# Rose-STL-Lab/spherical-dyffusion

Measured on AMD Instinct MI355X. Metric: forecast-steps/sec (180x360, 63ch), 25-member ensemble DYffusion sampling, whole job, higher is better.
Workload: dtype f32 tensors; every GEMM-class kernel (1x1 convs, fused MLP, Legendre analysis/synthesis, dhconv) as 3-pass split-f16 MFMA with f32 accumulation; FFT / norms / pointwise in f32 (statistics f64); 1 GPU; 25-member ensemble x horizon-6 DYffusion sampling pass (6 forecaster + 10 interpolator SFNO forwards, dropout stream on, AR feedback), 180x360, 63 state + 2 forcing channels, embed 256, 8 blocks; horizon=6, relayed_members=0, parallelism=members of one initial condition sharded over GPUs, no data-path collective

## Files before the change

spherical-dyffusion_amd/csrc/capi.hip:

```cpp
#include <cmath>
#include <cstdio>
#include <cstdlib>
#include <cstring>
#include <mutex>
#include <string>
#include <vector>

#include "common.h"
#include "fft.h"
#include "pointwise.h"

static inline int round_up(int v, int m) { return (v + m - 1) / m * m; }
static inline size_t round_up_sz(size_t v, size_t m) { return (v + m - 1) / m * m; }

template <class F>
static float h3_pack_host(std::vector<_Float16>& buf, int nb, int rows, int K, int rows_pad, int Kpad, F value) {
  float mx = 0.f;
  for (int b = 0; b < nb; ++b)
    for (int r = 0; r < rows; ++r)
      for (int k = 0; k < K; ++k) mx = std::fmax(mx, std::fabs(value(b, r, k)));
  const float s = sdy_h3_scale(mx);
  const size_t plane = (size_t)nb * rows_pad * Kpad;
  buf.assign(2 * plane, (_Float16)0.0f);
  for (int b = 0; b < nb; ++b)
// ... 50 lines not shown
  float* d_pct = nullptr;
  float* d_tw = nullptr;
  float* d_pw = nullptr;
  SdyFftDesc fft;
  int gemm_mode = 0;
  void* d_wq_h3 = nullptr;
  void* d_pct_h3 = nullptr;
  float s_wq = 1.f, s_pct = 1.f;
  int h3_rows_fwd = 0, h3_k_fwd = 0, h3_rows_inv = 0, h3_k_inv = 0;
  void* d_wq_frag = nullptr;
  void* d_pct_frag = nullptr;
  float s_wq_frag = 1.f, s_pct_frag = 1.f;
  void* d_wq_par = nullptr;
  void* d_pct_par = nullptr;
  float s_wq_par = 1.f, s_pct_par = 1.f;
  int* d_kdead = nullptr;
  int* d_mcut = nullptr;
  enum Leg { LEG_PAR, LEG_H3, LEG_GEMM_H3, LEG_GEMM_F32 } leg = LEG_GEMM_F32;
  bool fused360 = false;
};

namespace {
struct SdySwitches {
  bool gemm_f32, no_fft360, no_leg_par, no_leg_frag, no_dh_frag, no_fused_mlp, no_drop_skip, no_skip_fold;
};
const SdySwitches& sw() {
  static const SdySwitches v = [] {
    auto on = [](const char* n) { return std::getenv(n) != nullptr; };
    const char* g = std::getenv("SDY_GEMM_MODE");
    return SdySwitches{g && std::string(g) == "f32", on("SDY_NO_FFT360"), on("SDY_NO_LEG_PAR"), on("SDY_NO_LEG_FRAG"),
                       on("SDY_NO_DH_FRAG"), on("SDY_NO_FUSED_MLP"), on("SDY_NO_DROP_SKIP"), on("SDY_NO_SKIP_FOLD")};
  }();
  return v;
}
}
static int env_gemm_mode() { return sw().gemm_f32 ? 0 : 1; }

template <class D, class T>
static hipError_t upload(D** dst, const std::vector<T>& v) {
  hipError_t e = hipMalloc((void**)dst, v.size() * sizeof(T));
  return e == hipSuccess ? hipMemcpy(*dst, v.data(), v.size() * sizeof(T), hipMemcpyHostToDevice) : e;
}
struct LegTables { const float *wqT, *pf; int nlat, lmax, Lpad4, Kpad4; };
static float leg_wq_at(void* c, int m, int l, int k) {
  const LegTables* x = static_cast<const LegTables*>(c);
  return x->wqT[((size_t)m * x->nlat + k) * x->Lpad4 + l];
}
static float leg_pct_at(void* c, int m, int k, int l) {
  const LegTables* x = static_cast<const LegTables*>(c);
  return x->pf[((size_t)m * x->lmax + l) * x->Kpad4 + k];
}

extern "C" int sdy_sht_plan_create(int nlat, int nlon, int lmax, int mmax, int grid, sdy_sht_plan** out) {
  return sdy_sht_plan_create_ex(nlat, nlon, lmax, mmax, grid, env_gemm_mode(), out);
// ... 420 lines not shown
  if (!(p->fft.fft360 && p->fft.n == 180) || C % 16 != 0) return SDY_ERR_UNSUPPORTED;
  if (!tiled_stride_ok(zt_bstride, C, p->nlat * p->nlon)) return SDY_ERR_ARG;
  return sdy_fft360_launch_inv(p->fft, Yf, bias, nullptr, B, C, p->nlat, p->mtr, 0, nullptr, (hipStream_t)stream, zt, zt_bstride,
                               part);
}

static inline int h3_mpad(int Cout) { return Cout > 128 ? round_up(Cout, 256) : 128; }
static inline int h3_kpad(int Cin) { return round_up(Cin, 64); }

extern "C" size_t sdy_h3_pack_bytes(int Cout, int Cin) {
  if (Cout <= 0 || Cin <= 0) return 0;
  return (size_t)2 * h3_mpad(Cout) * h3_kpad(Cin) * sizeof(_Float16);
}

extern "C" int sdy_h3_pack_weight(const float* w, int Cout, int Cin, void* packed_dev, float* scale) {
  if (!w || !packed_dev || !scale || Cout <= 0 || Cin <= 0) return SDY_ERR_ARG;
  std::vector<_Float16> buf;
  *scale = h3_pack_host(buf, 1, Cout, Cin, h3_mpad(Cout), h3_kpad(Cin),
                        [&](int, int o, int i) { return w[(size_t)o * Cin + i]; });
  SDY_HIP_TRY(hipMemcpy(packed_dev, buf.data(), buf.size() * sizeof(_Float16), hipMemcpyHostToDevice));
  return SDY_OK;
}

extern "C" int sdy_conv1x1(const sdy_conv_args* a, void* stream) {
  if (!a || !a->x || (!a->wt && !a->w_h3 && !a->w_frag) || !a->out) return SDY_ERR_ARG;
  if (a->B <= 0 || a->Cin <= 0 || a->Cout <= 0 || a->HW <= 0) return SDY_ERR_ARG;
  if (!a->w_h3 && a->ldw < a->Cout) return SDY_ERR_ARG;
  if ((a->pa == nullptr) != (a->pd == nullptr)) return SDY_ERR_ARG;
  if (a->add_mode != 0 && !a->add) return SDY_ERR_ARG;
  if ((!a->w_h3 && (a->ldw & 3)) || (a->HW & 3) || (a->x_bstride & 3) || (a->out_bstride & 3)) return SDY_ERR_ALIGN;
  if (a->drop_p < 0.0f || a->drop_p >= 1.0f) return SDY_ERR_ARG;
  if (a->w_frag && sdy_conv256_h3_supported(a->Cin, a->Cout) && a->drop_p == 0.0f && !a->keep_mask && !a->batch_scale)
    return sdy_conv256_h3_launch(a, (hipStream_t)stream);
  if (a->stats || a->out_tiled || a->x_rows) return SDY_ERR_UNSUPPORTED;
  GemmParams g{};
  g.A = a->wt; g.lda = a->ldw; g.sA = 0;
  g.B = a->x; g.ldb = a->HW; g.sB = a->x_bstride;
  g.C = a->out; g.ldc = a->HW; g.sC = a->out_bstride;
  g.M = round_up(a->Cout, 4); g.M_store = a->Cout; g.N = a->HW; g.K = a->Cin; g.nbatch = a->B;
  g.tile = a->Cout > 64 ? SDY_TILE_128x128 : SDY_TILE_64x128;
  g.tag = (a->kernel_tag >= 1 && a->kernel_tag <= 3) ? a->kernel_tag : 0;
  g.pa = a->pa; g.pd = a->pd; g.p_bstride = a->Cin;
  g.bias = a->bias;
  g.add = a->add_mode ? a->add : nullptr; g.sAdd = a->add_bstride; g.ldadd = a->HW; g.add_mode = a->add_mode;
  g.act = a->act;
  if (a->drop_p > 0.0f) {
    g.drop_thr = sdy_drop_threshold16(a->drop_p);
    if (g.drop_thr == 0u) g.drop_thr = 1u;
    g.drop_scale = 1.0f / (1.0f - a->drop_p);
    g.keep_mask = a->keep_mask;
  }
  g.seed_lo = (uint32_t)(a->seed & 0xFFFFFFFFu); g.seed_hi = (uint32_t)(a->seed >> 32);
  g.stream_id = a->stream_id; g.call = a->call; g.batch_offset = a->batch_offset;
  if (a->rows_per_call < 0 || (a->rows_per_call > 0 && a->B % a->rows_per_call)) return SDY_ERR_ARG;
  g.rows_per_call = a->rows_per_call > 0 ? a->rows_per_call : a->B;
  g.batch_scale = a->batch_scale;
  if (a->w_h3) {
    const int Mp = h3_mpad(a->Cout), Kp = h3_kpad(a->Cin);
    return sdy_gemm_h3_launch(g, a->w_h3, Mp, Kp, 0, (long)Mp * Kp, a->w_h3_scale, 0, (hipStream_t)stream);
  }
  return sdy_gemm_launch(g, (hipStream_t)stream);
}

extern "C" int sdy_cold_update(const float* x_s, const float* x_ip_next, const float* x_ip_s, float* out, size_t n,
                               void* stream) {
  return sdy_cold_update_launch(x_s, x_ip_next, x_ip_s, out, n, (hipStream_t)stream);
}

extern "C" int sdy_concat_channels(const float* const* src, const int* chans, int nsrc, float* out, int B, int HW,
                                   void* stream) {
  if (!src || !chans || nsrc < 1 || nsrc > 4) return SDY_ERR_ARG;
  long total = 0;
  for (int i = 0; i < nsrc; ++i) total += chans[i];
  return sdy_concat_launch(src, chans, nsrc, out, total * HW, B, HW, (hipStream_t)stream);
}

extern "C" int sdy_cond_noise_fill(uint64_t seed, uint32_t call, uint32_t batch_offset, int rows_per_call, int B, int C, int HW,
                                   float* out, void* stream) {
  return sdy_cond_noise_launch(seed, call, batch_offset, rows_per_call, B, C, HW, out, (hipStream_t)stream);
}

namespace {

struct DevBuf {
  float* p = nullptr;
// ... 33 lines not shown
  if (c.gemm_mode != 1) return DH_GEMM_F32;
  if (!sdy_dhconv_frag_supported(c.embed_dim, c.embed_dim) || sw().no_dh_frag) return DH_GEMM_H3;
  return skip_foldable(c, i) && !sw().no_skip_fold ? DH_FOLDED : DH_FRAG;
}

namespace {
struct XfSide {
  const sdy_sht_plan* plan;
  bool polar;
  bool tiled;
  int ilv;
  const int* mcut;
};

struct BlockPath {
  XfSide in, out;
  bool scale_residual;
  bool fused_mlp;
  bool lazy_norm;
  bool cs_tiled;
  DhKind dh;
  enum Skip { SKIP_CONV, SKIP_GELU, SKIP_IN_FFT } skip;
  bool stats1;
  bool z_tiled;
  bool drop_skip;
};
}

struct sdy_sfno {
  sdy_sfno_config cfg;
  int HW, catC, decC, ldo;
  sdy_sht_plan* plan_data = nullptr;
  sdy_sht_plan* plan_lg = nullptr;
  DevBuf pos, e0w, e0b, e2w, d0w, d0b, d2w;
  struct Pair { std::vector<float> w1_host, w2_host; void* w = nullptr; float s1 = 1.0f, s2 = 1.0f; } enc, dec;
  DevBuf t1w, t1b, t3w, t3b, freq, wbt, bb;
  std::vector<BlockW> blk;
  std::vector<BlockPath> path;
  SdyTimeMlp tm;
  std::string missing;
  const float* enc_ws = nullptr;
  int enc_B = 0;
  bool enc_has_stats = false;
};

static int dev_alloc(DevBuf& b, size_t n) {
// ... 276 lines not shown
    if (rest == "mlp.fwd.2.bias" || rest == "mlp.fwd.3.bias") { EXPECT_NUMEL(E); return dev_upload(w.b2, host, numel); }
  }
  return SDY_ERR_NAME;
}

static BlockPath resolve_path(const sdy_sfno* n, int i) {
  const sdy_sfno_config& c = n->cfg;
  const BlockW& w = n->blk[i];
  const int E = c.embed_dim, ilv = spec_ilv(c);
  auto side = [&](const sdy_sht_plan* p) {
    const bool polar = plan_polar_ok(p, E), tiled = plan_tiled_ok(p, E, ilv);
    return XfSide{p, polar, tiled, tiled ? 2 : ilv, polar ? p->d_mcut : nullptr};
  };
  BlockPath b;
  b.in = side(i == 0 ? n->plan_data : n->plan_lg);
  b.out = side(i == c.num_layers - 1 ? n->plan_data : n->plan_lg);
  b.scale_residual = b.in.plan != b.out.plan;
  b.fused_mlp = w.mlp && !sw().no_fused_mlp;
  b.lazy_norm = b.fused_mlp && !b.scale_residual;
  b.dh = dhconv_kind(c, i);
  const bool dh_frag = b.dh == DH_FOLDED || b.dh == DH_FRAG;
  b.cs_tiled = b.in.tiled && b.out.tiled && dh_frag && b.in.plan->lmax == b.out.plan->lmax && b.in.plan->mtr == b.out.plan->mtr;
  b.stats1 = c.gemm_mode == 1 && w.skw.frag && sdy_conv256_h3_supported(E, E);
  b.z_tiled = b.stats1 && b.fused_mlp;
  b.skip = b.dh != DH_FOLDED ? BlockPath::SKIP_CONV : (b.out.tiled && b.z_tiled) ? BlockPath::SKIP_IN_FFT : BlockPath::SKIP_GELU;
  b.drop_skip = b.fused_mlp && b.z_tiled && b.cs_tiled && !sw().no_drop_skip;
  return b;
}

extern "C" int sdy_sfno_ready(const sdy_sfno* n_c) {
  sdy_sfno* n = const_cast<sdy_sfno*>(n_c);
  if (!n) return SDY_ERR_ARG;
  if (!n->path.empty()) return SDY_OK;
  const sdy_sfno_config& c = n->cfg;
  n->missing.clear();
  auto need = [&](const DevBuf& b, const std::string& nm) {
    if (!b.set && n->missing.empty()) n->missing = nm;
  };
  if (c.pos_embed) need(n->pos, "pos_embed");
  need(n->e0w, "encoder.0.weight"); need(n->e0b, "encoder.0.bias"); need(n->e2w, "encoder.2.weight");
  need(n->d0w, "decoder.0.weight"); need(n->d0b, "decoder.0.bias"); need(n->d2w, "decoder.2.weight");
  if (c.with_time_emb) {
    need(n->t1w, "time_emb_mlp.1.weight"); need(n->t1b, "time_emb_mlp.1.bias");
    need(n->t3w, "time_emb_mlp.3.weight"); need(n->t3b, "time_emb_mlp.3.bias");
  }
  for (int i = 0; i < c.num_layers; ++i) {
// ... 393 lines not shown
      SDY_STAGE_N(ST_FFT_INV, k.Bp, sdy_fft_launch_inv(pout->fft, Xf, bias, y, k.Bp, E, pout->nlat, pout->mtr, P.out.ilv,
                                                       P.out.mcut, stream));
    return SDY_OK;
  }

  int inner_skip(const Blk& k) {
    const BlockPath& P = k.P;
    const BlockW& bw = k.w;
    if (P.skip == BlockPath::SKIP_IN_FFT) {
      SDY_STAGE_N(ST_NORM_COEFFS, k.Bp, sdy_instnorm_from_partials_launch(sp, P.out.plan->nlat, k.Bp, E, HW, bw.n1w.p, bw.n1b.p,
                                                                          1e-6f, ca1, cd1, stream));
      return SDY_OK;
    }
    if (P.skip == BlockPath::SKIP_GELU) {
      SDY_STAGE_N(ST_SKIP_GELU, k.Bp, sdy_gelu_stats_launch(y, xbs, k.z, k.z_bs, P.z_tiled ? 1 : 0, st1, k.Bp, E, HW, stream));
    } else {
      sdy_conv_args cv = conv_args(bw.skw, k.Bp);
      cv.x_rows = P.lazy_norm ? k.rows : nullptr;
      cv.x = P.lazy_norm ? cur : xn; cv.x_bstride = xbs;
      if (P.lazy_norm) { cv.pa = ca; cv.pd = cd; }
      cv.ldw = E; cv.out = k.z; cv.out_bstride = k.z_bs; cv.out_tiled = P.z_tiled ? 1 : 0;
      cv.Cin = E; cv.Cout = E; cv.bias = bw.skb.p; cv.add = y; cv.add_bstride = xbs; cv.add_mode = 1; cv.act = 1; cv.kernel_tag = 3;
      if (P.stats1) cv.stats = st1;
      SDY_STAGE_N(ST_SKIP_CONV, k.Bp, sdy_conv1x1(&cv, stream));
    }
    if (P.skip == BlockPath::SKIP_GELU || P.stats1)
      SDY_STAGE_N(ST_NORM_COEFFS, k.Bp, sdy_instnorm_from_stats(st1, k.Bp, E, HW, bw.n1w.p, bw.n1b.p, nullptr, 0, 1e-6f, ca1, cd1,
                                                                stream));
    else
      SDY_STAGE(ST_NORM_COEFFS, sdy_instnorm_coeffs_launch(y, B, E, HW, bw.n1w.p, bw.n1b.p, nullptr, 0, 1e-6f, ca1, cd1, stream));
    return SDY_OK;
  }

  int mlp(const Blk& k) {
    const BlockW& bw = k.w;
    const int i = k.i, Hd = c.mlp_hidden;
    const float* dps = (drop && n->tm.dp_rate[i] > 0.f) ? dp + (size_t)i * B : nullptr;
    const float* keep1 = (pm > 0.f && a->keep_masks) ? a->keep_masks[2 * i] : nullptr;
    const float* keep2 = (pm > 0.f && a->keep_masks) ? a->keep_masks[2 * i + 1] : nullptr;
    if (k.P.fused_mlp) {
      sdy_mlp_args ma;
      std::memset(&ma, 0, sizeof(ma));
      ma.x = k.z; ma.x_bstride = k.z_bs; ma.x_tiled = k.P.z_tiled ? 1 : 0; ma.pa = ca1; ma.pd = cd1;
      ma.w = bw.mlp; ma.w1_scale = bw.mlp_s1; ma.w2_scale = bw.mlp_s2; ma.b1 = bw.b1.p; ma.b2 = bw.b2.p;
      ma.out = k.dst; ma.out_bstride = k.dst_bs;
      if (k.P.lazy_norm) { ma.add = cur; ma.add_bstride = xbs; ma.add_a = ca; ma.add_d = cd; }
      else { ma.add = xn; ma.add_bstride = xbs; ma.add_by_launch_row = k.rows ? 1 : 0; }
// ... 65 lines not shown
```

spherical-dyffusion_amd/csrc/common.h:

```cpp
#pragma once
#include <hip/hip_runtime.h>
#include <stdint.h>
#include <atomic>
#include <cmath>
#include <type_traits>

#include "../../include/sdy_amd.h"

#define SDY_HIP_TRY(expr)                       \
  do {                                          \
    hipError_t _e = (expr);                     \
    if (_e != hipSuccess) return (int)_e;       \
  } while (0)

#define SDY_TRY(expr)             \
  do {                            \
    int _r = (expr);              \
    if (_r != SDY_OK) return _r;  \
  } while (0)

static inline int sdy_launch_status() {
  hipError_t e = hipGetLastError();
  return e == hipSuccess ? SDY_OK : (int)e;
}
// ... 274 lines not shown
  int M_store;
  int lda, ldb, ldc;
  long sA, sB, sC;
  int nbatch;
  int a_kcontig;
  int b_cplx;
  int cplx_Ei, cplx_Eo;
  int tri_mode, tri_B;
  int tile;
  int tag;
  const float* pa; const float* pd; long p_bstride;
  const float* bias;
  const float* add; long sAdd; int ldadd; int add_mode;
  int act;
  uint32_t drop_thr; float drop_scale; const float* keep_mask;
  uint32_t seed_lo, seed_hi, stream_id, call, batch_offset;
  int rows_per_call;
  const float* batch_scale;
};
int sdy_gemm_launch(const GemmParams& p, hipStream_t stream);
int sdy_gemm_h3_launch(const GemmParams& p, const void* packed, int rows_pad, int Kpad, long bstride, long plane_halfs,
                       float w_scale, int rows_mode, hipStream_t stream);

int sdy_conv256_h3_launch(const sdy_conv_args* a, hipStream_t stream);
extern "C" int sdy_conv256_h3_pack_cin(const float* w_host, int Cin, void* dev, float* scale);
extern "C" size_t sdy_conv256_h3_pack_bytes_cin(int Cin);
int sdy_dh_h3_pack(const float* w_host, int L, void* packed_dev, float* scale, int ilv);
int sdy_dh_h3_launch(const float* Cs_in, const void* packed, float scale, float* Cs_out, int L, int mtr, int B, int ilv,
                      hipStream_t stream, int tiled = 0, int B_in = 0);

typedef float (*sdy_leg_value_fn)(void* ctx, int z, int row, int k);
int sdy_leg_h3_supported(int rows, int K);
size_t sdy_leg_h3_table_bytes(int nz);
int sdy_leg_h3_pack(int nz, int rows, int K, sdy_leg_value_fn value, void* ctx, void* dev, float* scale);
int sdy_leg_par_supported(int nlat, int lmax);
size_t sdy_leg_par_table_bytes(int nz);
int sdy_leg_par_pack(int nz, int nlat, int lmax, int fwd, sdy_leg_value_fn value, void* ctx, void* dev, float* scale);
int sdy_leg_par_launch(const void* table, float scale, int nz, const float* X, long ldx, long sX, float* C, long ldc,
                       long sC, int rows_out, int K, int N, int fwd, const int* kdead, hipStream_t stream, long tsx = 0, long tsc = 0);
int sdy_leg_h3_launch(const void* table, float scale, int nz, const float* X, long ldx, long sX, float* C, long ldc, long sC,
                      int M_store, int K, int N, int tri, hipStream_t stream);

int sdy_factor_radices(int n, int* radices, int* nstages);
```

spherical-dyffusion_amd/csrc/conv_h3.hip:

```cpp
#include <cmath>
#include <cstdlib>
#include <type_traits>
#include <vector>

#include "common.h"

namespace {

constexpr int CE = 256;
constexpr int CTN = 64;
constexpr int CKMAX = 384;
constexpr int CRING = 4;
constexpr float CSX = SDY_ACT_SX;
constexpr int CSTAT_BYTES = CE * 2 * 8;
#ifndef SDY_CONV_STAMP_T0
#define SDY_CONV_STAMP_T0 2
#endif

template <int KBLK, int NW>
struct ConvCfg {
  static_assert(NW == 4 || NW == 8, "4 or 8 waves");
  static constexpr int NT = 64 * NW;
  static constexpr int MT = 8 / NW;
  static constexpr int RS = 4 * NW;
// ... 16 lines not shown
  const float* x; long x_bs;
  const float* pa; const float* pd;
  const sdy_f16x8* w;
  const float* bias;
  const float* add; long add_bs; int add_mode;
  int act;
  float* out; long out_bs;
  int out_tiled;
  double* stats;
  int HW, B;
  int Cin;
  float out_scale;
  unsigned* flags;
  unsigned* head;
  const float* gelu_tab;
  SdyImgMap xmap;
  unsigned long long* stamps;
};

__device__ __forceinline__ int cv_swz(int px) { return (px & 15) ^ (((px >> 4) & 1) * 3); }
template <int KROW>
__device__ __forceinline__ int cv_off(int px, int c) { return px * KROW + (((c & ~15) | ((c ^ cv_swz(px)) & 15)) << 3); }

template <int KBLK, int NW>
__global__ __launch_bounds__(64 * NW, NW == 4 ? 2 : 1) void conv_h3_kernel(const ConvParams p) {
  using G = ConvCfg<KBLK, NW>;
  constexpr int CMT = G::MT, CRS = G::RS, COC = G::OC, CRPT = G::RPT, KROW = G::KROW, CGPK = G::GPK, CGPW = G::GPW;
  __shared__ __attribute__((aligned(16))) unsigned char smem[G::LDS_BYTES];
  _Float16* Xs_hi = reinterpret_cast<_Float16*>(smem);
  _Float16* Xs_lo = Xs_hi + CTN * KROW;
  float* Os = reinterpret_cast<float*>(smem);

  const int tid = threadIdx.x, lane = tid & 63, wave = tid >> 6;
  int h = lane >> 5, l31 = lane & 31;
  int q0 = tid & 15, o0 = tid >> 4;
  const int tpi = (p.HW + CTN - 1) / CTN;
  const int ntiles = tpi * p.B;
  const int t_per = (ntiles + (int)gridDim.x - 1) / (int)gridDim.x;
  const int t_begin = (int)blockIdx.x * t_per;
  const int t_end = (t_begin + t_per < ntiles) ? t_begin + t_per : ntiles;

  sdy_f16x8 r_hi[CRING], r_lo[CRING];
  constexpr int CGROUP_BYTES = SDY_GROUP * (int)sizeof(sdy_f16x8);
  const char* const wbase = reinterpret_cast<const char*>(p.w) + (size_t)__builtin_amdgcn_readfirstlane(wave) * CGPW * CGROUP_BYTES;
  unsigned woff = (unsigned)lane * 16u;
#pragma unroll
  for (int s = 0; s < CRING; ++s) {
    r_hi[s] = sdy_ring_ld(wbase, woff, 0);
    r_lo[s] = sdy_ring_ld(wbase, woff, CGROUP_BYTES / 2);
    woff += CGROUP_BYTES;
  }
  constexpr int NWIN = KBLK * CMT;
  if (NWIN == 1) woff -= CRING * CGROUP_BYTES;

  double* Ss = reinterpret_cast<double*>(smem + G::TILE_BYTES);
  float* Bs = reinterpret_cast<float*>(smem + G::TILE_BYTES + CSTAT_BYTES);
  if (tid < CE) {
    Bs[tid] = p.bias ? p.bias[tid] / p.out_scale : 0.0f;
    Ss[2 * tid] = 0.0; Ss[2 * tid + 1] = 0.0;
  }
  float* Gt = reinterpret_cast<float*>(smem + G::TILE_BYTES + CSTAT_BYTES + CE * 4);
  const unsigned gt_base = (unsigned)(uintptr_t)Gt;
  const bool tab_gelu = SDY_CONV_GELU_TAB && p.act == 1;
  if (tab_gelu) gelu_tab_to_lds(Gt, p.gelu_tab, tid, G::NT, 1.0f / SDY_GELU_SX);
  const float os_scale = tab_gelu ? p.out_scale * SDY_GELU_WS : p.out_scale;

  f32x4 xr[COC][8], addv[CRPT];
  auto img = [&](const float* base, long bs, int t) { return base + (long)(t / tpi) * bs; };
  auto ximg = [&](int t) { return p.x + (long)sdy_img(p.xmap, t / tpi) * p.x_bs; };
  auto lane_col = [&](int t) {
    const int nn = (t % tpi) * CTN + 4 * q0;
    return nn < p.HW ? nn : 0;
  };
  const float* addsrc = p.add ? p.add : p.out;
  const long addsrc_bs = p.add ? p.add_bs : p.out_bs;
  if (t_begin < t_end) {
    const float* xz = ximg(t_begin);
    const unsigned xo = (unsigned)(8 * o0 * p.HW + lane_col(t_begin)) * 4u;
#pragma unroll
    for (int oc = 0; oc < COC; ++oc)
#pragma unroll
      for (int e = 0; e < 8; ++e) {
        const int ch = 8 * (o0 + CRS * oc) + e;
        xr[oc][e] = f32x4{0.f, 0.f, 0.f, 0.f};
        if (ch < p.Cin) xr[oc][e] = sdy_ld16s(xz + (long)(8 * CRS * oc + e) * p.HW, xo);
      }
  }

  for (int tile = t_begin; tile < t_end; ++tile) {
    asm volatile("" : "+v"(l31), "+v"(h), "+v"(q0), "+v"(o0));
    const int tile_it = tile - t_begin;
    auto stamp = [&](int i) {
      if (SDY_STAMPS_ON && p.stamps && blockIdx.x == 3 && tid == 0 && tile_it >= SDY_CONV_STAMP_T0 && tile_it < SDY_CONV_STAMP_T0 + 4)
        p.stamps[(tile_it - SDY_CONV_STAMP_T0) * 8 + i] = __builtin_amdgcn_s_memtime();
    };
    stamp(0);
    const int z = tile / tpi;
    const int zx = sdy_img(p.xmap, z);
    const int n0 = (tile - z * tpi) * CTN;
    const bool full = n0 + CTN <= p.HW;

    {
      float amax = 0.0f;
      const bool ok = full || (n0 + 4 * q0 < p.HW);
#pragma unroll
      for (int oc = 0; oc < COC; ++oc) {
        const int c0 = 8 * (o0 + CRS * oc);
        if (8 * CRS * oc + 8 * CRS > KROW && c0 >= KROW) continue;
        float av[8], dv[8];
        if (p.pa) {
          const f32x4 a0 = *reinterpret_cast<const f32x4*>(p.pa + (long)zx * CE + c0);
          const f32x4 a1 = *reinterpret_cast<const f32x4*>(p.pa + (long)zx * CE + c0 + 4);
          const f32x4 d0 = *reinterpret_cast<const f32x4*>(p.pd + (long)zx * CE + c0);
          const f32x4 d1 = *reinterpret_cast<const f32x4*>(p.pd + (long)zx * CE + c0 + 4);
#pragma unroll
          for (int e = 0; e < 4; ++e) {
            av[e] = a0[e] * CSX; av[e + 4] = a1[e] * CSX;
            dv[e] = d0[e] * CSX; dv[e + 4] = d1[e] * CSX;
          }
        } else {
#pragma unroll
          for (int e = 0; e < 8; ++e) { av[e] = CSX; dv[e] = 0.f; }
        }
#pragma unroll
        for (int pp = 0; pp < 4; ++pp) {
          sdy_f16x8 vh, vl;
          float v[8];
#pragma unroll
          for (int e = 0; e < 8; ++e) v[e] = (ok && c0 + e < p.Cin) ? fmaf(xr[oc][e][pp], av[e], dv[e]) : 0.0f;
          sdy_split8(v, vh, vl, amax);
          const int off = cv_off<KROW>(4 * q0 + pp, o0 + CRS * oc);
          *reinterpret_cast<sdy_f16x8*>(Xs_hi + off) = vh;
          *reinterpret_cast<sdy_f16x8*>(Xs_lo + off) = vl;
        }
      }
      sdy_flag_range(p.flags, amax, p.head);
    }
    __syncthreads();
    stamp(1);
    const int col = n0 + 4 * q0;
    const bool c_ok = full || col < p.HW;
    const unsigned ro = (unsigned)(o0 * p.HW + (c_ok ? col : 0)) * 4u;
    const unsigned ro_out = p.out_tiled ? (unsigned)(o0 * CTN + 4 * q0) * 4u : ro;
    const int out_rs = p.out_tiled ? CTN : p.HW;
    const int tnext = (tile + 1 < t_end) ? tile + 1 : tile;
    const float* xz_next = ximg(tnext);
    const unsigned xo_next = (unsigned)(8 * o0 * p.HW + lane_col(tnext)) * 4u;
    stamp(2);
    f32x16 acc[CMT][2];
#pragma unroll
    for (int mi = 0; mi < CMT; ++mi)
#pragma unroll
      for (int r4 = 0; r4 < 4; ++r4) {
        const f32x4 b4 = *reinterpret_cast<const f32x4*>(Bs + 32 * (CMT * wave + mi) + 8 * r4 + 4 * h);
#pragma unroll
        for (int j = 0; j < 2; ++j)
#pragma unroll
          for (int r = 0; r < 4; ++r) acc[mi][j][4 * r4 + r] = b4[r];
      }
#pragma unroll
    for (int kb = 0; kb < KBLK; ++kb) {
#pragma unroll
      for (int i = 0; i < 4; ++i) {
        const int ks = 4 * kb + i;
        sdy_f16x8 bh[2], bl[2];
#pragma unroll
        for (int j = 0; j < 2; ++j) {
          const int off = cv_off<KROW>(32 * j + l31, 2 * ks + h);
          bh[j] = *reinterpret_cast<const sdy_f16x8*>(Xs_hi + off);
          bl[j] = *reinterpret_cast<const sdy_f16x8*>(Xs_lo + off);
        }
#pragma unroll
        for (int mi = 0; mi < CMT; ++mi) {
          const int g = kb * CGPK + CMT * i + mi;
          const int s = g % CRING;
#pragma unroll
          for (int j = 0; j < 2; ++j) SDY_CROSS_TERM(acc[mi][j] = __builtin_amdgcn_mfma_f32_32x32x16_f16(r_lo[s], bh[j], acc[mi][j], 0, 0, 0));
#pragma unroll
          for (int j = 0; j < 2; ++j) SDY_CROSS_TERM(acc[mi][j] = __builtin_amdgcn_mfma_f32_32x32x16_f16(r_hi[s], bl[j], acc[mi][j], 0, 0, 0));
#pragma unroll
          for (int j = 0; j < 2; ++j) acc[mi][j] = __builtin_amdgcn_mfma_f32_32x32x16_f16(r_hi[s], bh[j], acc[mi][j], 0, 0, 0);
          r_hi[s] = sdy_ring_ld(wbase, woff, 0);
          r_lo[s] = sdy_ring_ld(wbase, woff, CGROUP_BYTES / 2);
          woff += CGROUP_BYTES;
          if ((g + CRING + 1) % (NWIN * CRING) == 0) woff -= NWIN * CRING * CGROUP_BYTES;
          __builtin_amdgcn_sched_barrier(0);
        }
      }
    }

    stamp(3);
    {
      const float* az = img(addsrc, addsrc_bs, tile);
#pragma unroll
      for (int i = 0; i < CRPT; ++i) addv[i] = p.add ? sdy_ld16s(az + (long)(CRS * i) * p.HW, ro) : f32x4{0.f, 0.f, 0.f, 0.f};
    }
    __syncthreads();
    stamp(4);
#pragma unroll
    for (int mi = 0; mi < CMT; ++mi)
#pragma unroll
      for (int j = 0; j < 2; ++j)
#pragma unroll
        for (int r = 0; r < 16; ++r) {
          const int row = 32 * (CMT * wave + mi) + (r & 3) + 8 * (r >> 2) + 4 * h;
          Os[row * CTN + 32 * j + l31] = acc[mi][j][r] * os_scale;
        }
    __syncthreads();
    stamp(5);
    {
      float* oz = p.out + (long)z * p.out_bs + (p.out_tiled ? (long)(tile - z * tpi) * (CE * CTN) : 0L);
#pragma unroll
      for (int i = 0; i < CRPT; ++i) {
        f32x4 v = *reinterpret_cast<const f32x4*>(Os + (o0 + CRS * i) * CTN + 4 * q0);
        if (tab_gelu) {
          if (p.add_mode == 1) v = addv[i] * SDY_GELU_WS + v;
          v = f32x4{gelu_tab16(v.x, gt_base), gelu_tab16(v.y, gt_base), gelu_tab16(v.z, gt_base), gelu_tab16(v.w, gt_base)};
        } else {
        if (p.add_mode == 1) v += addv[i];
        if (p.act == 1) {
          const sdy_gf2 g0 = gelu_erf2(sdy_gf2{v.x, v.y}), g1 = gelu_erf2(sdy_gf2{v.z, v.w});
          v = f32x4{g0.x, g0.y, g1.x, g1.y};
        }
        }
        if (p.add_mode == 2) v += addv[i];
        if (c_ok) sdy_st16s(oz + (long)(CRS * i) * out_rs, ro_out, v);
#pragma unroll
        for (int k = 0; k < G::PPI; ++k) {
          const int piece = G::PPI * i + k, oc = piece >> 3, e = piece & 7;
          if (oc < COC) {
            const int ch = 8 * (o0 + CRS * oc) + e;
            if (ch < p.Cin) xr[oc][e] = sdy_ld16s(xz_next + (long)(8 * CRS * oc + e) * p.HW, xo_next);
          }
        }
        if (p.stats) {
          const float s1 = row16_sum(c_ok ? (v.x + v.y) + (v.z + v.w) : 0.0f);
          const float s2 = row16_sum(c_ok ? (v.x * v.x + v.y * v.y) + (v.z * v.z + v.w * v.w) : 0.0f);
          if (q0 == 0) {
            double* st = Ss + 2 * (o0 + CRS * i);
            __hip_atomic_fetch_add(st, (double)s1, __ATOMIC_RELAXED, __HIP_MEMORY_SCOPE_WORKGROUP);
            __hip_atomic_fetch_add(st + 1, (double)s2, __ATOMIC_RELAXED, __HIP_MEMORY_SCOPE_WORKGROUP);
          }
        }
      }
    }
    stamp(6);
    {
      const int nt = tile + 1;
      if (p.stats && (nt >= t_end || nt / tpi != z)) {
        __syncthreads();
        if (tid < CE) {
          double* st = p.stats + ((long)z * CE + tid) * 2;
          __hip_atomic_fetch_add(st, Ss[2 * tid], __ATOMIC_RELAXED, __HIP_MEMORY_SCOPE_AGENT);
          __hip_atomic_fetch_add(st + 1, Ss[2 * tid + 1], __ATOMIC_RELAXED, __HIP_MEMORY_SCOPE_AGENT);
          Ss[2 * tid] = 0.0; Ss[2 * tid + 1] = 0.0;
        }
      }
    }
    stamp(7);
    __syncthreads();
// ... 31 lines not shown
extern "C" int sdy_conv256_h3_pack_cin(const float* w_host, int Cin, void* dev, float* scale) {
  if (!w_host || !dev || !scale || Cin < 1 || Cin > CKMAX) return SDY_ERR_ARG;
  const float s = sdy_h3_scale(sdy_h3_absmax(w_host, (size_t)CE * Cin));
  int nw, ksw, mt;
  conv_layout(Cin, &nw, &ksw, &mt);
  const size_t gh = (size_t)SDY_GROUP * 8;
  std::vector<_Float16> buf((size_t)nw * mt * ksw * gh);
  _Float16* d = buf.data();
  for (int w = 0; w < nw; ++w)
    for (int ks = 0; ks < ksw; ++ks)
      for (int mi = 0; mi < mt; ++mi, d += gh)
        sdy_h3_put_group(d, s, [&](int r, int k) {
          const int kk = 16 * ks + k;
          return kk < Cin ? w_host[(size_t)(32 * (mt * w + mi) + r) * Cin + kk] : 0.0f;
        });
  SDY_HIP_TRY(hipMemcpy(dev, buf.data(), buf.size() * sizeof(_Float16), hipMemcpyHostToDevice));
  *scale = s;
  return SDY_OK;
}
extern "C" int sdy_conv256_h3_pack(const float* w_host, void* dev, float* scale) {
  return sdy_conv256_h3_pack_cin(w_host, CE, dev, scale);
}

template <int KBLK, int NW>
static void conv_launch(const ConvParams& p, long ntiles, int n_cu, hipStream_t stream) {
  using G = ConvCfg<KBLK, NW>;
  const long want = (long)n_cu * G::WGS;
  dim3 grid((unsigned)(ntiles < want ? ntiles : want));
  hipLaunchKernelGGL((conv_h3_kernel<KBLK, NW>), grid, dim3(G::NT), 0, stream, p);
}

int sdy_conv256_h3_launch(const sdy_conv_args* a, hipStream_t stream) {
  if (!a || !a->x || !a->w_frag || !a->out || a->B <= 0 || a->HW <= 0) return SDY_ERR_ARG;
  if (!sdy_conv256_h3_supported(a->Cin, a->Cout)) return SDY_ERR_UNSUPPORTED;
  if (a->drop_p > 0.f || a->keep_mask || a->batch_scale) return SDY_ERR_UNSUPPORTED;
  if (a->pa && a->Cin != CE) return SDY_ERR_UNSUPPORTED;
  if ((a->HW & 3) || (a->x_bstride & 3) || (a->out_bstride & 3) || (a->add_mode && (a->add_bstride & 3))) return SDY_ERR_ALIGN;
  if ((long)a->HW * CKMAX * 4 >= (1L << 32)) return SDY_ERR_UNSUPPORTED;
  ConvParams p;
  p.x = a->x; p.x_bs = a->x_bstride; p.pa = a->pa; p.pd = a->pd;
  p.w = reinterpret_cast<const sdy_f16x8*>(a->w_frag);
  p.bias = a->bias;
  p.add = a->add_mode ? a->add : nullptr; p.add_bs = a->add_bstride; p.add_mode = a->add_mode;
  p.act = a->act;
  p.out = a->out; p.out_bs = a->out_bstride; p.out_tiled = a->out_tiled;
  if (a->out_tiled && a->add_mode && a->add == a->out) return SDY_ERR_ARG;
  p.stats = a->stats;
  SDY_TRY(sdy_flags_ptr(&p.flags));
  SDY_TRY(sdy_headroom_ptr(SDY_RANGE_CONV, &p.head));
  SDY_TRY(sdy_gelu_table_ptr(&p.gelu_tab));
  p.HW = a->HW; p.B = a->B; p.Cin = a->Cin;
  SDY_TRY(sdy_img_map_fill(p.xmap, a->x_rows, a->B));
  p.out_scale = 1.0f / (a->w_frag_scale * CSX);
  p.stamps = nullptr;
#if SDY_STAMPS_ON
  if (std::getenv("SDY_CONV_STAMPS")) {
    if (!g_cstamps) SDY_HIP_TRY(hipMalloc(&g_cstamps, 64 * sizeof(unsigned long long)));
    p.stamps = g_cstamps;
  }
#endif
  int n_cu = 0;
  SDY_TRY(sdy_cu_count(&n_cu));
  const long ntiles = (long)((a->HW + CTN - 1) / CTN) * a->B;
  switch ((a->Cin + 63) / 64) {
    case 1: conv_launch<1, 4>(p, ntiles, n_cu, stream); break;
    case 2: conv_launch<2, 4>(p, ntiles, n_cu, stream); break;
    case 3: conv_launch<3, 4>(p, ntiles, n_cu, stream); break;
    case 4: conv_launch<4, 4>(p, ntiles, n_cu, stream); break;
    case 5: conv_launch<5, 8>(p, ntiles, n_cu, stream); break;
    default: conv_launch<6, 8>(p, ntiles, n_cu, stream); break;
  }
  return sdy_launch_status();
}
```

spherical-dyffusion_amd/ops.py:

```python
from __future__ import annotations

import ctypes as C
from typing import Optional

import torch

from ._lib import SdyConvArgs, SdyMlpArgs, SdyPairArgs, aligned, check, current_stream, lib, ptr


def _f32c(t: torch.Tensor) -> torch.Tensor:
    if not t.is_cuda:
        raise RuntimeError("sdy_amd ops run on the GPU only (no CPU fallback)")
    return aligned(t.to(torch.float32).contiguous())


def _aux(t: torch.Tensor, dev) -> torch.Tensor:
    return t.detach().to(dev, torch.float32).contiguous()


def contract_dhconv(x: torch.Tensor, weight: torch.Tensor, separable: bool = False,
                    operator_type: str = "dhconv", gemm_mode: Optional[str] = None) -> torch.Tensor:
    if separable or operator_type != "dhconv":
        raise NotImplementedError("only the non-separable dhconv contraction is on the hot path")
    B, Ci, L, M = x.shape
# ... 29 lines not shown
    out = out * tri[None, None, :, :, None]
    return torch.view_as_complex(out.contiguous())


def instnorm_coeffs(x: torch.Tensor, gamma: torch.Tensor, beta: torch.Tensor,
                    scale_shift: Optional[torch.Tensor] = None, eps: float = 1e-6):
    x = _f32c(x)
    B, Cc, H, W = x.shape
    a = torch.empty(B, Cc, dtype=torch.float32, device=x.device)
    d = torch.empty_like(a)
    g, b_ = _aux(gamma, x.device), _aux(beta, x.device)
    ss = _aux(scale_shift, x.device) if scale_shift is not None else None
    with torch.cuda.device(x.device):
        check(lib.sdy_instnorm_coeffs(ptr(x), B, Cc, H * W, ptr(g), ptr(b_), ptr(ss), 2 * Cc, eps, ptr(a), ptr(d),
                                      current_stream()), "sdy_instnorm_coeffs")
    return a, d


def conv1x1(x: torch.Tensor, weight: torch.Tensor, bias: Optional[torch.Tensor] = None, *,
            pre_affine=None, add: Optional[torch.Tensor] = None, add_mode: int = 0, gelu: bool = False,
            drop_p: float = 0.0, keep_mask: Optional[torch.Tensor] = None, seed: int = 0, call: int = 0,
            stream_id: int = 0, batch_offset: int = 0, batch_scale: Optional[torch.Tensor] = None,
            kernel_tag: int = 0, out: Optional[torch.Tensor] = None, wt_prepared=None, h3: bool = False,
            h3_prepared=None, frag_prepared=None, stats: Optional[torch.Tensor] = None) -> torch.Tensor:
    x = _f32c(x)
    B, Cin, H, W = x.shape
    w2 = weight.detach().to(torch.float32).reshape(weight.shape[0], -1)
    Cout = w2.shape[0]
    assert w2.shape[1] == Cin
    ldw = (Cout + 3) // 4 * 4
    if wt_prepared is not None:
        wt = wt_prepared
    else:
        wt = torch.zeros(Cin, ldw, dtype=torch.float32, device=x.device)
        wt[:, :Cout] = w2.t().to(x.device)
    if out is None:
        out = torch.empty(B, Cout, H, W, dtype=torch.float32, device=x.device)
    a = SdyConvArgs()
    a.x, a.x_bstride = ptr(x), Cin * H * W
    a.wt, a.ldw = ptr(wt), ldw
    a.out, a.out_bstride = ptr(out), Cout * H * W
    a.B, a.Cin, a.Cout, a.HW = B, Cin, Cout, H * W
    keep = [x, wt, out]
    if h3 or h3_prepared is not None:
        if h3_prepared is None:
            h3_prepared = pack_h3(w2, x.device)
        a.w_h3, a.w_h3_scale = ptr(h3_prepared[0]), h3_prepared[1]
        keep.append(h3_prepared[0])
    if pre_affine is not None:
        pa, pd = _aux(pre_affine[0], x.device), _aux(pre_affine[1], x.device)
        a.pa, a.pd = ptr(pa), ptr(pd)
        keep += [pa, pd]
    if bias is not None:
        bb = _aux(bias, x.device)
        a.bias = ptr(bb)
        keep.append(bb)
    if add is not None:
        ad = _aux(add, x.device)
        a.add = ptr(ad)
        a.add_bstride = 0 if ad.shape[0] == 1 and B > 1 else Cout * H * W
        a.add_mode = add_mode
        keep.append(ad)
    a.act = 1 if gelu else 0
    a.drop_p = drop_p
# ... 328 lines not shown
```

Baseline: 159.9 member-forecast-steps/s.

## Add weight-stationary 8-wave variant of the 256-channel split-f16 skip conv

Adds a weight-stationary specialization of the 256x256 conv_h3 kernel that runs on 8 waves. Each wave keeps its full slice of hi/lo weight fragments in registers for the whole K sweep, and B fragments from LDS are double-buffered across k-steps. The add and gelu/residual form is hard-wired, the residual load is moved before the MFMA loop, and the next tile's input is prefetched after it. This targets the skip conv in each block to cut repeated weight-ring reloads, at the cost of higher register pressure and one workgroup per CU. The Python wrapper also gains x_rows and out_tiled arguments.

```diff
diff --git a/spherical-dyffusion_amd/csrc/capi.hip b/spherical-dyffusion_amd/csrc/capi.hip
--- a/spherical-dyffusion_amd/csrc/capi.hip
+++ b/spherical-dyffusion_amd/csrc/capi.hip
@@ -96,14 +96,15 @@
 
 namespace {
 struct SdySwitches {
-  bool gemm_f32, no_fft360, no_leg_par, no_leg_frag, no_dh_frag, no_fused_mlp, no_drop_skip, no_skip_fold;
+  bool gemm_f32, no_fft360, no_leg_par, no_leg_frag, no_dh_frag, no_fused_mlp, no_drop_skip, no_skip_fold, no_conv_ws;
 };
 const SdySwitches& sw() {
   static const SdySwitches v = [] {
     auto on = [](const char* n) { return std::getenv(n) != nullptr; };
     const char* g = std::getenv("SDY_GEMM_MODE");
     return SdySwitches{g && std::string(g) == "f32", on("SDY_NO_FFT360"), on("SDY_NO_LEG_PAR"), on("SDY_NO_LEG_FRAG"),
-                       on("SDY_NO_DH_FRAG"), on("SDY_NO_FUSED_MLP"), on("SDY_NO_DROP_SKIP"), on("SDY_NO_SKIP_FOLD")};
+                       on("SDY_NO_DH_FRAG"), on("SDY_NO_FUSED_MLP"), on("SDY_NO_DROP_SKIP"), on("SDY_NO_SKIP_FOLD"),
+                       on("SDY_NO_CONV_WS")};
   }();
   return v;
 }
@@ -570,7 +571,7 @@
   return SDY_OK;
 }
 
-extern "C" int sdy_conv1x1(const sdy_conv_args* a, void* stream) {
+static int conv1x1(const sdy_conv_args* a, void* stream, bool conv_ws) {
   if (!a || !a->x || (!a->wt && !a->w_h3 && !a->w_frag) || !a->out) return SDY_ERR_ARG;
   if (a->B <= 0 || a->Cin <= 0 || a->Cout <= 0 || a->HW <= 0) return SDY_ERR_ARG;
   if (!a->w_h3 && a->ldw < a->Cout) return SDY_ERR_ARG;
@@ -579,7 +580,7 @@
   if ((!a->w_h3 && (a->ldw & 3)) || (a->HW & 3) || (a->x_bstride & 3) || (a->out_bstride & 3)) return SDY_ERR_ALIGN;
   if (a->drop_p < 0.0f || a->drop_p >= 1.0f) return SDY_ERR_ARG;
   if (a->w_frag && sdy_conv256_h3_supported(a->Cin, a->Cout) && a->drop_p == 0.0f && !a->keep_mask && !a->batch_scale)
-    return sdy_conv256_h3_launch(a, (hipStream_t)stream);
+    return sdy_conv256_h3_launch(a, (hipStream_t)stream, conv_ws ? 1 : 0);
   if (a->stats || a->out_tiled || a->x_rows) return SDY_ERR_UNSUPPORTED;
   GemmParams g{};
   g.A = a->wt; g.lda = a->ldw; g.sA = 0;
@@ -609,6 +610,7 @@
   }
   return sdy_gemm_launch(g, (hipStream_t)stream);
 }
+extern "C" int sdy_conv1x1(const sdy_conv_args* a, void* stream) { return conv1x1(a, stream, !sw().no_conv_ws); }
 
 extern "C" int sdy_cold_update(const float* x_s, const float* x_ip_next, const float* x_ip_s, float* out, size_t n,
                                void* stream) {
@@ -688,6 +690,7 @@
   DhKind dh;
   enum Skip { SKIP_CONV, SKIP_GELU, SKIP_IN_FFT } skip;
   bool stats1;
+  bool conv_ws;
   bool z_tiled;
   bool drop_skip;
 };
@@ -1010,6 +1013,7 @@
   const bool dh_frag = b.dh == DH_FOLDED || b.dh == DH_FRAG;
   b.cs_tiled = b.in.tiled && b.out.tiled && dh_frag && b.in.plan->lmax == b.out.plan->lmax && b.in.plan->mtr == b.out.plan->mtr;
   b.stats1 = c.gemm_mode == 1 && w.skw.frag && sdy_conv256_h3_supported(E, E);
+  b.conv_ws = b.stats1 && !sw().no_conv_ws;
   b.z_tiled = b.stats1 && b.fused_mlp;
   b.skip = b.dh != DH_FOLDED ? BlockPath::SKIP_CONV : (b.out.tiled && b.z_tiled) ? BlockPath::SKIP_IN_FFT : BlockPath::SKIP_GELU;
   b.drop_skip = b.fused_mlp && b.z_tiled && b.cs_tiled && !sw().no_drop_skip;
@@ -1449,7 +1453,7 @@
       cv.ldw = E; cv.out = k.z; cv.out_bstride = k.z_bs; cv.out_tiled = P.z_tiled ? 1 : 0;
       cv.Cin = E; cv.Cout = E; cv.bias = bw.skb.p; cv.add = y; cv.add_bstride = xbs; cv.add_mode = 1; cv.act = 1; cv.kernel_tag = 3;
       if (P.stats1) cv.stats = st1;
-      SDY_STAGE_N(ST_SKIP_CONV, k.Bp, sdy_conv1x1(&cv, stream));
+      SDY_STAGE_N(ST_SKIP_CONV, k.Bp, conv1x1(&cv, stream, P.conv_ws));
     }
     if (P.skip == BlockPath::SKIP_GELU || P.stats1)
       SDY_STAGE_N(ST_NORM_COEFFS, k.Bp, sdy_instnorm_from_stats(st1, k.Bp, E, HW, bw.n1w.p, bw.n1b.p, nullptr, 0, 1e-6f, ca1, cd1,
diff --git a/spherical-dyffusion_amd/csrc/common.h b/spherical-dyffusion_amd/csrc/common.h
--- a/spherical-dyffusion_amd/csrc/common.h
+++ b/spherical-dyffusion_amd/csrc/common.h
@@ -320,7 +320,8 @@
 int sdy_gemm_h3_launch(const GemmParams& p, const void* packed, int rows_pad, int Kpad, long bstride, long plane_halfs,
                        float w_scale, int rows_mode, hipStream_t stream);
 
-int sdy_conv256_h3_launch(const sdy_conv_args* a, hipStream_t stream);
+int sdy_conv256_h3_launch(const sdy_conv_args* a, hipStream_t stream, int ws);
+int sdy_conv256_h3_ws_form(const sdy_conv_args* a);
 extern "C" int sdy_conv256_h3_pack_cin(const float* w_host, int Cin, void* dev, float* scale);
 extern "C" size_t sdy_conv256_h3_pack_bytes_cin(int Cin);
 int sdy_dh_h3_pack(const float* w_host, int L, void* packed_dev, float* scale, int ilv);
diff --git a/spherical-dyffusion_amd/csrc/conv_h3.hip b/spherical-dyffusion_amd/csrc/conv_h3.hip
--- a/spherical-dyffusion_amd/csrc/conv_h3.hip
+++ b/spherical-dyffusion_amd/csrc/conv_h3.hip
@@ -62,9 +62,11 @@
 template <int KROW>
 __device__ __forceinline__ int cv_off(int px, int c) { return px * KROW + (((c & ~15) | ((c ^ cv_swz(px)) & 15)) << 3); }
 
-template <int KBLK, int NW>
+template <int KBLK, int NW, bool WS = false>
 __global__ __launch_bounds__(64 * NW, NW == 4 ? 2 : 1) void conv_h3_kernel(const ConvParams p) {
   using G = ConvCfg<KBLK, NW>;
+  static_assert(!WS || (KBLK == 4 && NW == 8), "weight-stationary: 256 input channels on 8 waves");
+  constexpr int RING = WS ? G::KSW : CRING;
   constexpr int CMT = G::MT, CRS = G::RS, COC = G::OC, CRPT = G::RPT, KROW = G::KROW, CGPK = G::GPK, CGPW = G::GPW;
   __shared__ __attribute__((aligned(16))) unsigned char smem[G::LDS_BYTES];
   _Float16* Xs_hi = reinterpret_cast<_Float16*>(smem);
@@ -72,6 +74,9 @@
   float* Os = reinterpret_cast<float*>(smem);
 
   const int tid = threadIdx.x, lane = tid & 63, wave = tid >> 6;
+  auto Cin = [&] { return WS ? CE : p.Cin; };
+  auto add_mode = [&] { return WS ? 1 : p.add_mode; };
+  auto act = [&] { return WS ? 1 : p.act; };
   int h = lane >> 5, l31 = lane & 31;
   int q0 = tid & 15, o0 = tid >> 4;
   const int tpi = (p.HW + CTN - 1) / CTN;
@@ -80,18 +85,20 @@
   const int t_begin = (int)blockIdx.x * t_per;
   const int t_end = (t_begin + t_per < ntiles) ? t_begin + t_per : ntiles;
 
-  sdy_f16x8 r_hi[CRING], r_lo[CRING];
+  sdy_f16x8 r_hi[RING], r_lo[RING];
   constexpr int CGROUP_BYTES = SDY_GROUP * (int)sizeof(sdy_f16x8);
-  const char* const wbase = reinterpret_cast<const char*>(p.w) + (size_t)__builtin_amdgcn_readfirstlane(wave) * CGPW * CGROUP_BYTES;
+  const int uwave = __builtin_amdgcn_readfirstlane(wave);
+  const char* const wbase = reinterpret_cast<const char*>(p.w) +
+                            (WS ? (size_t)((uwave >> 1) * 2 * G::KSW + (uwave & 1)) * CGROUP_BYTES : (size_t)uwave * CGPW * CGROUP_BYTES);
   unsigned woff = (unsigned)lane * 16u;
 #pragma unroll
-  for (int s = 0; s < CRING; ++s) {
+  for (int s = 0; s < RING; ++s) {
     r_hi[s] = sdy_ring_ld(wbase, woff, 0);
     r_lo[s] = sdy_ring_ld(wbase, woff, CGROUP_BYTES / 2);
-    woff += CGROUP_BYTES;
+    woff += (WS ? 2 : 1) * CGROUP_BYTES;
   }
   constexpr int NWIN = KBLK * CMT;
-  if (NWIN == 1) woff -= CRING * CGROUP_BYTES;
+  if (!WS && NWIN == 1) woff -= CRING * CGROUP_BYTES;
 
   double* Ss = reinterpret_cast<double*>(smem + G::TILE_BYTES);
   float* Bs = reinterpret_cast<float*>(smem + G::TILE_BYTES + CSTAT_BYTES);
@@ -101,7 +108,7 @@
   }
   float* Gt = reinterpret_cast<float*>(smem + G::TILE_BYTES + CSTAT_BYTES + CE * 4);
   const unsigned gt_base = (unsigned)(uintptr_t)Gt;
-  const bool tab_gelu = SDY_CONV_GELU_TAB && p.act == 1;
+  const bool tab_gelu = SDY_CONV_GELU_TAB && act() == 1;
   if (tab_gelu) gelu_tab_to_lds(Gt, p.gelu_tab, tid, G::NT, 1.0f / SDY_GELU_SX);
   const float os_scale = tab_gelu ? p.out_scale * SDY_GELU_WS : p.out_scale;
 
@@ -123,7 +130,7 @@
       for (int e = 0; e < 8; ++e) {
         const int ch = 8 * (o0 + CRS * oc) + e;
         xr[oc][e] = f32x4{0.f, 0.f, 0.f, 0.f};
-        if (ch < p.Cin) xr[oc][e] = sdy_ld16s(xz + (long)(8 * CRS * oc + e) * p.HW, xo);
+        if (WS || ch < Cin()) xr[oc][e] = sdy_ld16s(xz + (long)(8 * CRS * oc + e) * p.HW, xo);
       }
   }
 
@@ -167,7 +174,7 @@
           sdy_f16x8 vh, vl;
           float v[8];
 #pragma unroll
-          for (int e = 0; e < 8; ++e) v[e] = (ok && c0 + e < p.Cin) ? fmaf(xr[oc][e][pp], av[e], dv[e]) : 0.0f;
+          for (int e = 0; e < 8; ++e) v[e] = (ok && (WS || c0 + e < Cin())) ? fmaf(xr[oc][e][pp], av[e], dv[e]) : 0.0f;
           sdy_split8(v, vh, vl, amax);
           const int off = cv_off<KROW>(4 * q0 + pp, o0 + CRS * oc);
           *reinterpret_cast<sdy_f16x8*>(Xs_hi + off) = vh;
@@ -186,6 +193,12 @@
     const int tnext = (tile + 1 < t_end) ? tile + 1 : tile;
     const float* xz_next = ximg(tnext);
     const unsigned xo_next = (unsigned)(8 * o0 * p.HW + lane_col(tnext)) * 4u;
+    if constexpr (WS) {
+      const float* az = img(p.add, p.add_bs, tile);
+#pragma unroll
+      for (int i = 0; i < CRPT; ++i) addv[i] = sdy_ld16s(az + (long)(CRS * i) * p.HW, ro);
+      __builtin_amdgcn_sched_barrier(0);
+    }
     stamp(2);
     f32x16 acc[CMT][2];
 #pragma unroll
@@ -198,18 +211,36 @@
 #pragma unroll
           for (int r = 0; r < 4; ++r) acc[mi][j][4 * r4 + r] = b4[r];
       }
+    auto ld_b = [&](int ks, sdy_f16x8* bh, sdy_f16x8* bl) {
+#pragma unroll
+      for (int j = 0; j < 2; ++j) {
+        const int off = cv_off<KROW>(32 * j + l31, 2 * ks + h);
+        bh[j] = *reinterpret_cast<const sdy_f16x8*>(Xs_hi + off);
+        bl[j] = *reinterpret_cast<const sdy_f16x8*>(Xs_lo + off);
+      }
+    };
+    if constexpr (WS) {
+      sdy_f16x8 bh[2][2], bl[2][2];
+      ld_b(0, bh[0], bl[0]);
+      sdy_static_for<0, G::KSW>([&](auto ks_c) {
+        constexpr int ks = decltype(ks_c)::value, c = ks & 1;
+        if constexpr (ks + 1 < G::KSW) ld_b(ks + 1, bh[c ^ 1], bl[c ^ 1]);
+#pragma unroll
+        for (int j = 0; j < 2; ++j) SDY_CROSS_TERM(acc[0][j] = __builtin_amdgcn_mfma_f32_32x32x16_f16(r_lo[ks], bh[c][j], acc[0][j], 0, 0, 0));
+#pragma unroll
+        for (int j = 0; j < 2; ++j) SDY_CROSS_TERM(acc[0][j] = __builtin_amdgcn_mfma_f32_32x32x16_f16(r_hi[ks], bl[c][j], acc[0][j], 0, 0, 0));
+#pragma unroll
+        for (int j = 0; j < 2; ++j) acc[0][j] = __builtin_amdgcn_mfma_f32_32x32x16_f16(r_hi[ks], bh[c][j], acc[0][j], 0, 0, 0);
+        __builtin_amdgcn_sched_barrier(0);
+      });
+    } else {
 #pragma unroll
     for (int kb = 0; kb < KBLK; ++kb) {
 #pragma unroll
       for (int i = 0; i < 4; ++i) {
         const int ks = 4 * kb + i;
         sdy_f16x8 bh[2], bl[2];
-#pragma unroll
-        for (int j = 0; j < 2; ++j) {
-          const int off = cv_off<KROW>(32 * j + l31, 2 * ks + h);
-          bh[j] = *reinterpret_cast<const sdy_f16x8*>(Xs_hi + off);
-          bl[j] = *reinterpret_cast<const sdy_f16x8*>(Xs_lo + off);
-        }
+        ld_b(ks, bh, bl);
 #pragma unroll
         for (int mi = 0; mi < CMT; ++mi) {
           const int g = kb * CGPK + CMT * i + mi;
@@ -228,9 +259,15 @@
         }
       }
     }
+    }
 
     stamp(3);
-    {
+    if constexpr (WS) {
+      static_assert(!WS || COC == 1, "one channel octet per thread");
+#pragma unroll
+      for (int e = 0; e < 8; ++e) xr[0][e] = sdy_ld16s(xz_next + (long)e * p.HW, xo_next);
+      __builtin_amdgcn_sched_barrier(0);
+    } else {
       const float* az = img(addsrc, addsrc_bs, tile);
 #pragma unroll
       for (int i = 0; i < CRPT; ++i) addv[i] = p.add ? sdy_ld16s(az + (long)(CRS * i) * p.HW, ro) : f32x4{0.f, 0.f, 0.f, 0.f};
@@ -254,28 +291,29 @@
       for (int i = 0; i < CRPT; ++i) {
         f32x4 v = *reinterpret_cast<const f32x4*>(Os + (o0 + CRS * i) * CTN + 4 * q0);
         if (tab_gelu) {
-          if (p.add_mode == 1) v = addv[i] * SDY_GELU_WS + v;
+          if (add_mode() == 1) v = addv[i] * SDY_GELU_WS + v;
           v = f32x4{gelu_tab16(v.x, gt_base), gelu_tab16(v.y, gt_base), gelu_tab16(v.z, gt_base), gelu_tab16(v.w, gt_base)};
         } else {
-        if (p.add_mode == 1) v += addv[i];
-        if (p.act == 1) {
+        if (add_mode() == 1) v += addv[i];
+        if (act() == 1) {
           const sdy_gf2 g0 = gelu_erf2(sdy_gf2{v.x, v.y}), g1 = gelu_erf2(sdy_gf2{v.z, v.w});
           v = f32x4{g0.x, g0.y, g1.x, g1.y};
         }
         }
-        if (p.add_mode == 2) v += addv[i];
+        if (add_mode() == 2) v += addv[i];
         if (c_ok) sdy_st16s(oz + (long)(CRS * i) * out_rs, ro_out, v);
 #pragma unroll
         for (int k = 0; k < G::PPI; ++k) {
           const int piece = G::PPI * i + k, oc = piece >> 3, e = piece & 7;
           if (oc < COC) {
             const int ch = 8 * (o0 + CRS * oc) + e;
-            if (ch < p.Cin) xr[oc][e] = sdy_ld16s(xz_next + (long)(8 * CRS * oc + e) * p.HW, xo_next);
+            if constexpr (!WS)
+              if (ch < Cin()) xr[oc][e] = sdy_ld16s(xz_next + (long)(8 * CRS * oc + e) * p.HW, xo_next);
           }
         }
         if (p.stats) {
-          const float s1 = row16_sum(c_ok ? (v.x + v.y) + (v.z + v.w) : 0.0f);
-          const float s2 = row16_sum(c_ok ? (v.x * v.x + v.y * v.y) + (v.z * v.z + v.w * v.w) : 0.0f);
+          const float s1 = row16_sum(c_ok ? sdy_quad_sum(v) : 0.0f);
+          const float s2 = row16_sum(c_ok ? sdy_quad_sumsq(v) : 0.0f);
           if (q0 == 0) {
             double* st = Ss + 2 * (o0 + CRS * i);
             __hip_atomic_fetch_add(st, (double)s1, __ATOMIC_RELAXED, __HIP_MEMORY_SCOPE_WORKGROUP);
@@ -353,15 +391,19 @@
   return sdy_conv256_h3_pack_cin(w_host, CE, dev, scale);
 }
 
-template <int KBLK, int NW>
+template <int KBLK, int NW, bool WS = false>
 static void conv_launch(const ConvParams& p, long ntiles, int n_cu, hipStream_t stream) {
   using G = ConvCfg<KBLK, NW>;
   const long want = (long)n_cu * G::WGS;
   dim3 grid((unsigned)(ntiles < want ? ntiles : want));
-  hipLaunchKernelGGL((conv_h3_kernel<KBLK, NW>), grid, dim3(G::NT), 0, stream, p);
-}
-
-int sdy_conv256_h3_launch(const sdy_conv_args* a, hipStream_t stream) {
+  hipLaunchKernelGGL((conv_h3_kernel<KBLK, NW, WS>), grid, dim3(G::NT), 0, stream, p);
+}
+
+int sdy_conv256_h3_ws_form(const sdy_conv_args* a) {
+  return a && SDY_CONV_GELU_TAB && a->Cin == CE && a->Cout == CE && a->add_mode == 1 && a->add && a->act == 1;
+}
+
+int sdy_conv256_h3_launch(const sdy_conv_args* a, hipStream_t stream, int ws) {
   if (!a || !a->x || !a->w_frag || !a->out || a->B <= 0 || a->HW <= 0) return SDY_ERR_ARG;
   if (!sdy_conv256_h3_supported(a->Cin, a->Cout)) return SDY_ERR_UNSUPPORTED;
   if (a->drop_p > 0.f || a->keep_mask || a->batch_scale) return SDY_ERR_UNSUPPORTED;
@@ -397,7 +439,10 @@
     case 1: conv_launch<1, 4>(p, ntiles, n_cu, stream); break;
     case 2: conv_launch<2, 4>(p, ntiles, n_cu, stream); break;
     case 3: conv_launch<3, 4>(p, ntiles, n_cu, stream); break;
-    case 4: conv_launch<4, 4>(p, ntiles, n_cu, stream); break;
+    case 4:
+      if (ws && sdy_conv256_h3_ws_form(a)) conv_launch<4, 8, true>(p, ntiles, n_cu, stream);
+      else conv_launch<4, 4>(p, ntiles, n_cu, stream);
+      break;
     case 5: conv_launch<5, 8>(p, ntiles, n_cu, stream); break;
     default: conv_launch<6, 8>(p, ntiles, n_cu, stream); break;
   }
diff --git a/spherical-dyffusion_amd/ops.py b/spherical-dyffusion_amd/ops.py
--- a/spherical-dyffusion_amd/ops.py
+++ b/spherical-dyffusion_amd/ops.py
@@ -75,9 +75,15 @@
             drop_p: float = 0.0, keep_mask: Optional[torch.Tensor] = None, seed: int = 0, call: int = 0,
             stream_id: int = 0, batch_offset: int = 0, batch_scale: Optional[torch.Tensor] = None,
             kernel_tag: int = 0, out: Optional[torch.Tensor] = None, wt_prepared=None, h3: bool = False,
-            h3_prepared=None, frag_prepared=None, stats: Optional[torch.Tensor] = None) -> torch.Tensor:
+            h3_prepared=None, frag_prepared=None, stats: Optional[torch.Tensor] = None,
+            x_rows=None, out_tiled: bool = False) -> torch.Tensor:
     x = _f32c(x)
     B, Cin, H, W = x.shape
+    rows_host = None
+    if x_rows is not None:
+        assert all(0 <= int(r) < B for r in x_rows)
+        rows_host = (C.c_ubyte * len(x_rows))(*[int(r) for r in x_rows])
+        B = len(x_rows)
     w2 = weight.detach().to(torch.float32).reshape(weight.shape[0], -1)
     Cout = w2.shape[0]
     assert w2.shape[1] == Cin
@@ -88,11 +94,15 @@
         wt = torch.zeros(Cin, ldw, dtype=torch.float32, device=x.device)
         wt[:, :Cout] = w2.t().to(x.device)
     if out is None:
-        out = torch.empty(B, Cout, H, W, dtype=torch.float32, device=x.device)
+        shape = (B, (H * W + 63) // 64, Cout, 64) if out_tiled else (B, Cout, H, W)
+        out = torch.empty(shape, dtype=torch.float32, device=x.device)
     a = SdyConvArgs()
     a.x, a.x_bstride = ptr(x), Cin * H * W
     a.wt, a.ldw = ptr(wt), ldw
-    a.out, a.out_bstride = ptr(out), Cout * H * W
+    a.out, a.out_bstride = ptr(out), out.numel() // B if out_tiled else Cout * H * W
+    a.out_tiled = 1 if out_tiled else 0
+    if rows_host is not None:
+        a.x_rows = C.addressof(rows_host)
     a.B, a.Cin, a.Cout, a.HW = B, Cin, Cout, H * W
     keep = [x, wt, out]
     if h3 or h3_prepared is not None:
```

After: 161.9 member-forecast-steps/s (median of 6 runs). +1.3%, better.
